# nmdp-bioinformatics/py-graph-imputation

Measured on AMD Instinct MI355X. Metric: imputed subjects/sec (whole node), 5-locus CAU graph, higher is better.
Workload: dtype f64; 1 GPU; BASELINE configs[1]: CAU 5-locus graph, 10k synthetic fully-typed subjects; 10000 subjects per step and GPU, seed=rank; graph_nodes=35411, populations=1

## Files before the change

py-graph-imputation_amd/csrc/grim_engine.hip:

```cpp
#include <hip/hip_runtime.h>
#include <hip/hip_ext.h>
#include <stdio.h>
#include <stdlib.h>
#include <string.h>
#include <algorithm>
#include <atomic>
#include <mutex>
#include <string>
#include <vector>

#include "grim_plan_a.h"
#include "grim_plan_b.h"
#include "grim_small.h"
#include "grim_medium.h"
#include "grim_mid.h"
#include "grim_tables.h"
#include "grim_tokdev.h"
#include "grim_em.h"
#include "grim_refresh.h"
#include "grim_marginal.h"
#include "grim_match.h"
#include "grim_search.h"
#include "grim_engine_internal.h"
#include "grim_host_internal.h"
// ... 492 lines not shown
  g->rf_short.clear();
  g->rf_long.clear();
  uint32_t pos = 0;
  for (uint32_t v = 0; v < V; ++v) {
    const uint32_t m = d->node_mask[v];
    if (m == d->full_mask) continue;
    const std::string node = "partial node " + std::to_string(v);
    if (m >= (1u << GRIM_MAXL)) return no(node + ": label mask beyond GRIM_MAXL");
    const uint32_t lo = d->a_start[v], hi = v + 1 < V ? d->a_start[v + 1] : n_a;
    if (lo != pos) return no(node + ": its top-link row does not begin where the row before it ends");
    if (hi <= lo) return no(node + ": empty top-link row");
    if (hi > n_a) return no(node + ": its top-link row ends beyond the links");
    for (uint32_t e = lo; e < hi; ++e) {
      const uint32_t r = d->a_nbr[e];
      if (r >= V || d->node_mask[r] != d->full_mask) return no(node + ": a top link that does not end at a full node");
      if ((d->node_key[r] & slots[m]) != d->node_key[v]) return no(node + ": a top link to a full haplotype that does not project onto it");
    }
    (hi - lo <= RF_SHORT_MAX ? g->rf_short : g->rf_long).push_back(v);
    pos = hi;
  }
  if (pos != n_a) return no("top links beyond the rows of the partial nodes");
  g->refreshable = true;
  g->refresh_why.clear();
  g->n_a_nbr = n_a;
  g->full_first = f_lo;
  g->n_full = f_hi - f_lo;
}

extern "C" grim_graph *grim_graph_upload(grim_ctx *c, const grim_graph_desc *d) {
  if (!c || !d) return nullptr;
  hipSetDevice(c->device);
  if (d->n_pops == 0 || d->n_pops > GRIM_MAXPOP) { set_err(c, "grim_graph_upload: population count out of range"); return nullptr; }
  if (d->n_loci == 0 || d->n_loci > GRIM_MAXL) { set_err(c, "grim_graph_upload: locus count out of range"); return nullptr; }
  if (d->n_nodes >= (1u << 23)) { set_err(c, "grim_graph_upload: more than 2^23 nodes"); return nullptr; }
  grim_graph *g = new grim_graph();
  g->ctx = c;
  g->bytes = 0;
  uint32_t cap = 64;
  static const int ht_factor = getenv("GRIM_HT_FACTOR") ? atoi(getenv("GRIM_HT_FACTOR")) : 0;
  while (cap < (uint64_t)(ht_factor > 1 ? ht_factor : (d->n_nodes > (1u << 18) ? 4 : 2)) * (uint64_t)d->n_nodes) cap <<= 1;
  std::vector<uint64_t> hk(cap, 0);
  std::vector<uint32_t> hv(cap, 0);
  bool unique_names = true;
  for (uint32_t i = 0; i < d->n_nodes; ++i) {
    uint64_t k = d->node_key[i];
    if (k == 0) { set_err(c, "grim_graph_upload: node with empty key"); delete g; return nullptr; }
    uint32_t h = (uint32_t)host_mix64(k) & (cap - 1);
    while (hk[h] != 0 && hk[h] != k) h = (h + 1) & (cap - 1);
    if (hk[h] == k) unique_names = false;
    hk[h] = k;
    hv[h] = i;
  }
  uint32_t max_deg = 0;
  for (uint32_t i = 0; i < d->n_nodes; ++i)
    if (d->a_start[i + 1] > d->a_start[i]) max_deg = std::max(max_deg, d->a_start[i + 1] - d->a_start[i]);
  uint32_t maxlab = 0;
  for (uint32_t m = 0; m < (1u << GRIM_MAXL); ++m) {
    uint32_t n = d->lab_start[m + 1] - d->lab_start[m];
    if (n > maxlab) maxlab = n;
  }
  g->max_label = maxlab;
  DevGraph &D = g->d;
  D.n_nodes = d->n_nodes;
  D.P = d->n_pops;
  D.n_loci = d->n_loci;
  D.full_mask = d->full_mask;
  D.ht_mask = cap - 1;
  D.n_conn = d->n_conn;
  D.node_key = upload(c, g->bufs, d->node_key, d->n_nodes, &g->bytes);
  D.node_mask = upload(c, g->bufs, d->node_mask, d->n_nodes, &g->bytes);
  D.freq = upload(c, g->bufs, d->freq, (size_t)d->n_nodes * d->n_pops, &g->bytes);
  D.a_start = upload(c, g->bufs, d->a_start, (size_t)d->n_nodes + 1, &g->bytes);
  D.a_nbr = upload(c, g->bufs, d->a_nbr, d->n_a_nbr, &g->bytes);
  D.b_conn = upload(c, g->bufs, d->b_conn, (size_t)d->n_nodes * GRIM_MAXL, &g->bytes);
  D.b_start = upload(c, g->bufs, d->b_start, (size_t)d->n_conn + 1, &g->bytes);
  D.b_nbr = upload(c, g->bufs, d->b_nbr, d->n_b_nbr, &g->bytes);
  D.lab_start = upload(c, g->bufs, d->lab_start, (1u << GRIM_MAXL) + 1, &g->bytes);
  D.lab_nodes = upload(c, g->bufs, d->lab_nodes, d->n_nodes, &g->bytes);
  {
    std::vector<uint64_t> lk(d->n_nodes);
    for (uint32_t i = 0; i < d->n_nodes; ++i) lk[i] = d->node_key[d->lab_nodes[i]];
    D.lab_key = upload(c, g->bufs, lk.data(), d->n_nodes, &g->bytes);
  }
  D.scan_ok = (unique_names && max_deg < (1u << 22) && d->n_pops <= 64) ? 1u : 0u;
  D.order_bad = d->label_order_bad;
  {
    std::vector<HtEnt> ht(cap);
    for (uint32_t i = 0; i < cap; ++i) {
      ht[i].key = hk[i];
      ht[i].val = hv[i];
      ht[i].pad = 0;
    }
    D.ht = upload(c, g->bufs, ht.data(), cap, &g->bytes);
  }
  {
    uint32_t nfull = d->lab_start[d->full_mask + 1] - d->lab_start[d->full_mask];
    uint32_t fcap = 64;
    static const int fht_factor = getenv("GRIM_FHT_FACTOR") ? atoi(getenv("GRIM_FHT_FACTOR")) : 8;
    while (fcap < (uint64_t)(fht_factor > 1 ? fht_factor : 2) * (uint64_t)nfull) fcap <<= 1;
    std::vector<FullEnt> ft(fcap);
    memset(ft.data(), 0, sizeof(FullEnt) * fcap);
    for (uint32_t i = 0; i < d->n_nodes; ++i) {
      if (d->node_mask[i] != d->full_mask) continue;
      uint64_t k = d->node_key[i];
      uint32_t h = fht_hash(k) & (fcap - 1);
      while (ft[h].key != 0 && ft[h].key != k) h = (h + 1) & (fcap - 1);
      ft[h].key = k;
      ft[h].f0 = d->freq[(size_t)i * d->n_pops];
    }
    D.fht = upload(c, g->bufs, ft.data(), fcap, &g->bytes);
    D.fht_mask = fcap - 1;
  }
  if (!D.fht || !D.node_key || !D.node_mask || !D.freq || !D.a_start || !D.a_nbr || !D.b_conn || !D.b_start || !D.b_nbr ||
      !D.lab_start || !D.lab_nodes || !D.lab_key || !D.ht) {
    set_err(c, "grim_graph_upload: device allocation or copy failed");
    for (void *p : g->bufs) hipFree(p);
    delete g;
    return nullptr;
  }
  refresh_check_rows(g, d);
  return g;
}

static void refresh_state_free(RefreshState *rf);

extern "C" void grim_graph_free(grim_graph *g) {
  if (!g) return;
  hipSetDevice(g->ctx->device);
  refresh_state_free(g->rf);
  for (void *p : g->bufs) hipFree(p);
  delete g;
}

extern "C" uint64_t grim_graph_device_bytes(const grim_graph *g) { return g ? g->bytes : 0; }


static uint64_t align256(uint64_t x) { return (x + 255) & ~255ull; }

static thread_local int tl_device = -1;
static inline void use_device(int dev) {
  if (tl_device != dev) {
    hipSetDevice(dev);
    tl_device = dev;
  }
}

static int env_int(const char *name, int dflt) {
  const char *v = getenv(name);
  return v ? atoi(v) : dflt;
}

uint32_t engine_small_stride(const grim_params *p) { return GRIM_SMALL_ROWS_FIXED + (p->n_results < 16 ? p->n_results : 16); }

uint64_t engine_rows_per_subject(const grim_params *p, uint32_t P) {
  return 2ull * p->n_results + 2ull * (p->n_pop_results < (uint64_t)P * P ? p->n_pop_results : (uint64_t)P * P);
}

static bool dev_realloc(uint8_t *&ptr, uint64_t bytes) {
  if (ptr) hipFree(ptr);
  ptr = nullptr;
  return hipMalloc((void **)&ptr, bytes ? bytes : 256) == hipSuccess;
}
static bool pin_realloc(uint8_t *&ptr, uint64_t bytes) {
  if (ptr) hipHostFree(ptr);
  ptr = nullptr;
  return hipHostMalloc((void **)&ptr, bytes ? bytes : 256, hipHostMallocDefault) == hipSuccess;
}

static std::atomic<uint64_t> g_moved[2];

static bool batch_plan(grim_batch *b, const EnginePlan &pl) {
  const uint64_t n = pl.n_subj ? pl.n_subj : 1;
  uint64_t o = 0;
  auto take = [&](uint64_t bytes) { uint64_t r = o; o = align256(o + bytes); return r; };
  const uint64_t o_state = take(8ull * (GRIM_NCTR + GRIM_NQ / 2));
  const bool devtok = pl.text_cap != 0;
  const uint64_t o_lines = take(devtok ? sizeof(LineRec) * n : 0), o_text = take(devtok ? pl.text_cap + 64 : 0);
  const uint64_t o_subj = take(sizeof(grim_subject) * n);
  const uint64_t o_small = take(sizeof(SmallRec) * n);
  const uint64_t o_os = take(4 * n), o_om = take(4 * n), o_og = take(4 * n);
  const uint64_t o_tok = take(2 * ((pl.tok_cap ? pl.tok_cap : 1) + (devtok ? (uint64_t)TOK_LANES * n : 0)));
  const uint64_t in_bytes = o;
  o = 0;
  const uint64_t small_waves = ((n + GRIM_WG / 32 - 1) / (GRIM_WG / 32)) * (GRIM_WG / 64);
  const uint64_t w_bail = take(4 * n), w_next = take(4 * n), w_ctr = take(4 * (4 * small_waves + 4));
  const uint64_t w_mid = take(4 * n);
  const uint64_t w_dsmall = take(devtok ? sizeof(SmallRec) * n : 0);
  const uint64_t w_t1 = take(sizeof(TabWork) * 2 * n), w_t2 = take(sizeof(TabWork) * 2 * n);
  const uint64_t work_bytes = o;
  o = 0;
  const uint64_t o_res = take(sizeof(grim_subject_result) * n);
  const uint64_t o_rows = take(sizeof(grim_row) * b->row_limit);
  const uint64_t out_bytes = o;
  bool ok = true;
  if (in_bytes > b->in_cap || !b->d_in) {
    const uint64_t want = in_bytes > b->in_cap ? in_bytes : b->in_cap;
    ok = ok && dev_realloc(b->d_in, want) && pin_realloc(b->h_in, want);
    b->in_cap = ok ? want : 0;
  }
  if (work_bytes > b->work_cap || !b->d_work) {
    const uint64_t want = work_bytes > b->work_cap ? work_bytes : b->work_cap;
    ok = ok && dev_realloc(b->d_work, want);
    b->work_cap = ok ? want : 0;
  }
  if (out_bytes > b->out_cap || !b->d_out) {
    const uint64_t want = out_bytes > b->out_cap ? out_bytes : b->out_cap;
    ok = ok && dev_realloc(b->d_out, want);
    b->out_cap = ok ? want : 0;
  }
  if (!ok) return false;
  b->plan = pl;
  b->off_tok = o_tok;
  b->off_rows = o_rows;
  DevArgs &A = b->a;
  A.counters = (unsigned long long *)(b->d_in + o_state);
  A.queue = (uint32_t *)(A.counters + GRIM_NCTR);
  A.row_head = A.queue + 1;
  A.next_count = A.queue + 2;
  A.subj = (const grim_subject *)(b->d_in + o_subj);
  b->d_small = (SmallRec *)(b->d_in + o_small);
  b->d_lines = devtok ? (LineRec *)(b->d_in + o_lines) : nullptr;
  b->d_text = devtok ? b->d_in + o_text : nullptr;
  b->d_dsmall = devtok ? (SmallRec *)(b->d_work + w_dsmall) : nullptr;
  b->off_subj = o_subj;
  b->h.lines = devtok ? (LineRec *)(b->h_in + o_lines) : nullptr;
  b->h.text = devtok ? b->h_in + o_text : nullptr;
  b->d_os = (uint32_t *)(b->d_in + o_os);
  b->d_om = (uint32_t *)(b->d_in + o_om);
  A.order = (const uint32_t *)(b->d_in + o_og);
  A.tok = (const uint16_t *)(b->d_in + o_tok);
  A.bail_list = (uint32_t *)(b->d_work + w_bail);
  A.next_list = (uint32_t *)(b->d_work + w_next);
  {
    static const int no_mid = env_int("GRIM_NO_MID", 0);
    A.mid_list = no_mid ? nullptr : (uint32_t *)(b->d_work + w_mid);
  }
  A.small_ctr = (uint32_t *)(b->d_work + w_ctr);
  A.t1_list = (TabWork *)(b->d_work + w_t1);
  A.t2_list = (TabWork *)(b->d_work + w_t2);
  A.res = (grim_subject_result *)(b->d_out + o_res);
  A.rows = (grim_row *)(b->d_out + o_rows);
  A.row_cap = (uint32_t)b->row_limit;
  A.priors = b->d_priors;
  A.next_cap = (uint32_t)n;
  b->h.subj = (grim_subject *)(b->h_in + o_subj);
  b->h.small = (SmallRec *)(b->h_in + o_small);
  b->h.order_s = (uint32_t *)(b->h_in + o_os);
  b->h.order_m = (uint32_t *)(b->h_in + o_om);
  b->h.order_g = (uint32_t *)(b->h_in + o_og);
  b->h.tok = (uint16_t *)(b->h_in + o_tok);
  b->h.res = (grim_subject_result *)b->h_out;
  b->h.rows = (grim_row *)(b->h_out ? b->h_out + o_rows : nullptr);
  return true;
}

static void batch_init_params(grim_batch *b, const grim_graph *g, const grim_params *p) {
  b->g = g;
  DevArgs &A = b->a;
  A.g = g->d;
  A.prm = *p;
  const uint32_t P = g->d.P;
  b->small_stride = engine_small_stride(p);
  A.pair_cap = GRIM_MAXPH * p->top_n * p->top_n;
  uint32_t tab = 64;
  while (tab < 2 * A.pair_cap) tab <<= 1;
  A.tab_cap = tab;
  A.bset_cap = g->max_label;
  SlotLayout &L = A.lay;
  uint64_t o = 0;
  auto take = [&](uint64_t n) { uint64_t r = o; o = align256(o + n); return r; };
  L.Tp = take(8ull * GRIM_SIDES * GRIM_TOPCAP);
  L.Tm = take(8ull * GRIM_SIDES * GRIM_TOPCAP);
  L.Te = take(4ull * GRIM_SIDES * GRIM_TOPCAP);
  L.k0 = take(8ull * tab);
  L.k1 = take(8ull * tab);
  L.tmin = take(4ull * tab);
  L.tgid = take(4ull * tab);
  L.Useq = take(4ull * A.pair_cap);
  L.Uprob = take(8ull * A.pair_cap);
  L.Uslot = take(4ull * A.pair_cap);
  L.ska = take(8ull * A.pair_cap);
  L.skb = take(8ull * A.pair_cap);
  L.sva = take(4ull * A.pair_cap);
  L.svb = take(4ull * A.pair_cap);
  L.gsum = take(8ull * A.pair_cap);
  L.ghead = take(4ull * A.pair_cap);
  L.gstart = take(4ull * (A.pair_cap + 1));
  L.gcnt = take(4ull * (A.pair_cap > P * P ? A.pair_cap : P * P));
  L.qsum = take(8ull * P * P);
  L.qfirst = take(4ull * P * P);
  L.bset = take(4ull * GRIM_NWAVE * GRIM_MAXL * (uint64_t)A.bset_cap);
  L.comp = take(8ull * GRIM_COMP_CAP);
  {
    uint32_t pc = 64;
    while (pc < 2 * A.bset_cap) pc <<= 1;
    A.proj_cap = pc;
  }
  L.proj_k = take(8ull * GRIM_NWAVE * A.proj_cap);
  L.proj_p = take(4ull * GRIM_NWAVE * A.proj_cap);
  L.rtok = take(2ull * GRIM_RTOK_CAP);
  L.save = take(p->save_mode ? 8ull * GRIM_NWAVE * 2 * GRIM_SAVE_CAP * (P + 1) : 0);
  L.stride = align256(o);
  b->timing = env_int("GRIM_TIMING", 0) != 0;
  A.flags = (env_int("GRIM_TABLES_HBM", 0) ? GRIM_F_TABLES_HBM : 0u) | (env_int("GRIM_NO_NODUP", 0) ? GRIM_F_NO_NODUP : 0u) |
            (env_int("GRIM_NO_SIDEMASK", 0) ? GRIM_F_NO_SIDEMASK : 0u);
  memset(b->acc_ms, 0, sizeof(b->acc_ms));
  b->n_timed = 0;
  b->n_subj = b->n_small = b->n_medium = b->n_general = 0;
  b->rows_used = 0;
}

grim_batch *engine_batch_create(grim_ctx *c, const grim_graph *g, const grim_params *p, uint64_t row_limit, const EnginePlan *plan) {
  if (!c || !g || !p || !plan) return nullptr;
  use_device(c->device);
  if (p->top_n == 0 || p->top_n > GRIM_TOPCAP) { set_err(c, "grim_batch_upload: max_haplotypes_number_in_phase must be 1..128"); return nullptr; }
  if (p->n_ladder < 0 || p->n_ladder > GRIM_MAXLADDER) { set_err(c, "grim_batch_upload: epsilon ladder too long"); return nullptr; }
  if (row_limit > 0x7FFFFFF0ull) row_limit = 0x7FFFFFF0ull;
  if (row_limit < 64) row_limit = 64;
  grim_batch *b = nullptr;
  if (!c->spare.empty()) {
    b = c->spare.back();
    c->spare.pop_back();
    if (b->d_priors) hipFree(b->d_priors);
    if (b->h_priors) hipHostFree(b->h_priors);
    b->d_priors = b->h_priors = nullptr;
    b->priors_cap = b->priors_up = 0;
  } else {
    b = new grim_batch();
    memset((void *)b, 0, sizeof(*b));
    b->ctx = c;
    bool ok = true;
    if (hipHostMalloc((void **)&b->hstate, 8 * (GRIM_NCTR + GRIM_NQ / 2)) != hipSuccess) {
      b->hstate = nullptr;
      ok = false;
    }
    for (auto &pair : b->ev)
      for (hipEvent_t &e : pair) ok = ok && hipEventCreate(&e) == hipSuccess;
    ok = ok && hipEventCreateWithFlags(&b->ev_done, hipEventDisableTiming | hipEventReleaseToSystem) == hipSuccess;
// ... 62 lines not shown
  use_device(c->device);
  grim_devdict *dd = new grim_devdict();
  dd->ctx = c;
  memset(&dd->d, 0, sizeof(dd->d));
  dd->d.n_loci = snap->n_loci;
  for (uint32_t s = 0; s < GRIM_MAXL; ++s) dd->d.locus_len[s] = 0xFFFFFFFFu;
  for (const DictSnap::Locus &L : snap->loci) {
    if (L.slot >= GRIM_MAXL || L.name.empty() || L.name.size() > 8) continue;
    uint64_t v = 0;
    for (size_t k = 0; k < L.name.size(); ++k) v |= (uint64_t)(uint8_t)L.name[k] << (56 - 8 * k);
    dd->d.locus[L.slot] = v;
    dd->d.locus_len[L.slot] = (uint32_t)L.name.size();
  }
  bool ok = true;
  for (uint32_t s = 0; s < snap->n_loci && s < GRIM_MAXL && ok; ++s) {
    const uint32_t cnt = snap->base[s];
    uint32_t cap = 16;
    while (cap < 4ull * cnt) cap <<= 1;
    std::vector<DictEnt> tab(cap);
    memset(tab.data(), 0, sizeof(DictEnt) * cap);
    for (uint32_t id = 0; id < cnt; ++id) {
      const sv nm = snap->name(s, id);
      if (nm.empty() || nm.size() > GRIM_TOKNAME) continue;
      DictEnt e;
      pack_name(nm.data(), nm.size(), e.w);
      e.hash = tokname_hash(e.w, (uint32_t)nm.size());
      e.meta = 0x80000000u | ((uint32_t)nm.size() << 16) | (id & 0xFFFFu);
      uint32_t k = e.hash & (cap - 1);
      while (tab[k].meta >> 31) k = (k + 1) & (cap - 1);
      tab[k] = e;
    }
    DictEnt *dt = upload(c, dd->bufs, tab.data(), cap, nullptr);
    ok = dt != nullptr;
    dd->d.tab[s] = dt;
    dd->d.mask[s] = cap - 1;
  }
  if (!ok) {
    set_err(c, "engine_devdict_create: device allocation or copy failed");
    engine_devdict_free(dd);
    return nullptr;
  }
  return dd;
}

void engine_devdict_free(grim_devdict *d) {
  if (!d) return;
  use_device(d->ctx->device);
  for (void *p : d->bufs) hipFree(p);
  delete d;
}

void engine_batch_set_dict(grim_batch *b, const grim_devdict *d) {
  if (b) b->dict = d;
}

uint32_t engine_batch_irregular(const grim_batch *b) { return b ? b->n_irregular : 0; }
uint32_t engine_graph_order_bad(const grim_graph *g) { return g ? g->d.order_bad : 0; }

int engine_batch_grow_pool(grim_batch *b, uint64_t max_records) {
  if (!b || b->pool_asked <= b->a.ppool_cap) return 0;
  uint64_t want = b->pool_asked + b->pool_asked / 8 + 4096;
  if (want > max_records || want > 0x7FFFFFF0ull) return 0;
  if (want <= b->pool_want) return 0;
  b->pool_want = want;
  return 1;
}

static int batch_set_rows(grim_batch *b, uint64_t rows) {
  const uint64_t old = b->row_limit;
  b->row_limit = rows;
  const EnginePlan pl = b->plan;
  if (!batch_plan(b, pl)) {
    (void)hipGetLastError();
    b->row_limit = old;
    if (!batch_plan(b, pl)) set_err(b->ctx, "grim_batch: device allocation failed while growing the row pool");
    return 0;
  }
  return 1;
}
int engine_batch_grow_rows(grim_batch *b, uint64_t max_rows) {
  if (!b || b->rows_used < b->a.row_cap || b->row_limit >= max_rows) return 0;
  use_device(b->ctx->device);
  uint64_t want = b->row_limit * 2;
  if (want > max_rows) want = max_rows;
  if (want > 0x7FFFFFF0ull) want = 0x7FFFFFF0ull;
  if (want <= b->row_limit) return 0;
  return batch_set_rows(b, want);
}
uint64_t engine_batch_row_limit(const grim_batch *b) { return b ? b->row_limit : 0; }
void engine_batch_hint_rows(grim_batch *b, uint64_t rows) {
  if (!b || rows <= b->row_limit) return;
  use_device(b->ctx->device);
  (void)batch_set_rows(b, rows);
}

uint64_t engine_batch_pool_want(const grim_batch *b) { return b ? b->pool_want : 0; }
void engine_batch_hint_pool(grim_batch *b, uint64_t records) {
  if (b && records > b->pool_want) b->pool_want = records;
}

int engine_batch_load(grim_batch *b, const EngineLoad *ld) {
  if (!b || !ld) return -1;
  grim_ctx *c = b->ctx;
  use_device(c->device);
  DevArgs &A = b->a;
  b->ran_ok = false;
  if (ld->n_subj > b->plan.n_subj || ld->tok_used > b->plan.tok_cap) {
    set_err(c, "engine_batch_load: beyond what the batch was planned for");
    return -1;
  }
  hipStream_t st = c->stream;
  const uint32_t P = b->g->d.P;
  const uint64_t PP = (uint64_t)P * P;
  if (ld->priors && (ld->n_priors != b->priors_up || !b->d_priors)) {
    if (ld->n_priors + 1 > b->priors_cap || !b->d_priors) {
      const uint32_t want = ld->n_priors + 1 > 2 * b->priors_cap ? ld->n_priors + 1 : 2 * b->priors_cap;
      if (b->d_priors) hipFree(b->d_priors);
      if (b->h_priors) hipHostFree(b->h_priors);
      b->d_priors = b->h_priors = nullptr;
      if (hipMalloc((void **)&b->d_priors, 8 * (uint64_t)want * PP) != hipSuccess ||
          hipHostMalloc((void **)&b->h_priors, 8 * (uint64_t)want * PP, hipHostMallocDefault) != hipSuccess) {
        set_err(c, "engine_batch_load: allocation of the prior matrices failed");
        return -1;
      }
      b->priors_cap = want;
    }
    if (ld->n_priors) memcpy(b->h_priors, ld->priors, 8 * (uint64_t)ld->n_priors * PP);
    for (uint64_t k = 0; k < PP; ++k) b->h_priors[(uint64_t)ld->n_priors * PP + k] = 1.0;
    HIPCHK(hipMemcpyAsync(b->d_priors, b->h_priors, 8 * ((uint64_t)ld->n_priors + 1) * PP, hipMemcpyHostToDevice, st), c, -1);
    g_moved[0] += 8 * ((uint64_t)ld->n_priors + 1) * PP;
    b->priors_up = ld->n_priors;
  }
  A.priors = b->d_priors;
  A.ones_prior = b->priors_up;
  if (ld->dev_hi > ld->dev_lo && (!b->dict || !b->d_lines || ld->text_bytes > b->plan.text_cap || ld->dev_hi > ld->n_subj)) {
    set_err(c, "engine_batch_load: the batch was not planned for the device tokenizer");
    return -1;
  }
  b->dev_lo = ld->dev_lo;
  b->dev_hi = ld->dev_hi;
  b->n_dev_lines = ld->dev_hi > ld->dev_lo ? ld->dev_hi - ld->dev_lo : 0;
  b->n_irregular = 0;
  b->n_subj = ld->n_subj;
  b->n_small = ld->n_small;
  b->n_medium = ld->n_medium;
  b->n_general = ld->n_general;
  b->last_load = *ld;
  b->last_load.priors = nullptr;
  A.n_medium = ld->n_medium;
  A.n_work = ld->n_general;
  unsigned long long *hs = (unsigned long long *)b->h_in;
  memset(hs, 0, 8 * (GRIM_NCTR + GRIM_NQ / 2));
  {
    const uint64_t staged = ((uint64_t)b->n_small + b->n_dev_lines) * b->small_stride;
    A.row_cap = (uint32_t)(b->row_limit - (staged <= b->row_limit ? staged : 0));
  }
  const bool host_subjects = ld->n_small + ld->n_medium + ld->n_general > 0;
  const uint64_t bytes = (!host_subjects && b->n_dev_lines) ? b->off_subj : b->off_tok + 2 * ld->tok_used;
  HIPCHK(hipMemcpyAsync(b->d_in, b->h_in, bytes, hipMemcpyHostToDevice, c->up_stream), c, -1);
  HIPCHK(hipEventRecord(b->ev_up, c->up_stream), c, -1);
  b->up_pending = true;
  g_moved[0] += bytes;
  {
    uint64_t R = (1ull << 20) + 512ull * ((uint64_t)ld->n_medium + ld->n_general) + 16ull * ld->n_small;
    R += (uint64_t)(ld->n_general < 256u ? ld->n_general : 256u) * (A.pair_cap / 2);
    const char *env_pool = getenv("GRIM_PAIR_POOL");
    if (env_pool && atol(env_pool) > 0) R = (uint64_t)atol(env_pool);
    if (b->pool_want > R) R = b->pool_want;
    if (R > 0x7FFFFFF0ull) R = 0x7FFFFFF0ull;
    const uint64_t items = 2ull * ld->n_subj < R / 256 + 1 ? 2ull * ld->n_subj : R / 256 + 1;
    uint64_t cap_b = R / 4 + (items + 1) * ((uint64_t)P * P + 4), cap_u = R / 4 + items * 64 + 1024;
    if (cap_b > R + 4096) cap_b = R + 4096;
    uint64_t o = 0;
    auto take = [&](uint64_t bytes) { uint64_t r = o; o = align256(o + bytes); return r; };
    const uint64_t o_pool = take(sizeof(PairRec) * R), o_aux = take(sizeof(TabAux) * 2 * (uint64_t)(ld->n_subj ? ld->n_subj : 1)),
                   o_boff = take(4 * cap_b), o_cell = take(sizeof(CellRec) * cap_b), o_units = take(sizeof(TabUnit) * cap_u),
                   o_sort = take(4 * 3 * R), o_grp = take(sizeof(GrpRec) * 2 * R), o_prob = take(8 * R);
    if (o > b->pool_bytes || !b->d_pool) {
      HIPCHK(hipStreamSynchronize(st), c, -1);
      if (b->d_pool) hipFree(b->d_pool);
      b->d_pool = nullptr;
      b->pool_bytes = 0;
      if (hipMalloc((void **)&b->d_pool, o) != hipSuccess) {
        (void)hipGetLastError();
        set_err(c, "engine_batch_load: cannot allocate " + std::to_string((unsigned long long)(o >> 20)) + " MiB for the table kernels");
        return -1;
      }
      b->pool_bytes = o;
    }
    b->pool_cap = R;
    A.ppool = (PairRec *)(b->d_pool + o_pool);
    A.ppool_cap = (uint32_t)R;
    A.taux = (TabAux *)(b->d_pool + o_aux);
    A.tboff = (uint32_t *)(b->d_pool + o_boff);
    A.tcell = (CellRec *)(b->d_pool + o_cell);
    A.tboff_cap = (uint32_t)cap_b;
    A.tunits = (TabUnit *)(b->d_pool + o_units);
    A.tunits_cap = (uint32_t)cap_u;
    A.tstride = (uint32_t)R;
    A.psort = (uint32_t *)(b->d_pool + o_sort);
    A.pgrp = (GrpRec *)(b->d_pool + o_grp);
    A.pprob = (double *)(b->d_pool + o_prob);
  }
  const uint32_t per_block = GRIM_WG / 32;
  b->n_host_small_waves = ((b->n_small + per_block - 1) / per_block) * (GRIM_WG / 64);
  b->n_small_waves = b->n_host_small_waves + ((b->n_dev_lines + per_block - 1) / per_block) * (GRIM_WG / 64);
  uint32_t slots = (uint32_t)c->n_cu * GRIM_WG_PER_CU;
  static const int env_slots = env_int("GRIM_SLOTS", 0);
  if (env_slots > 0) slots = (uint32_t)env_slots;
  if (slots > ld->n_subj) slots = ld->n_subj;
  if (slots == 0) slots = 1;
  b->n_slots = slots;
  b->scratch_need = (uint64_t)A.lay.stride * slots;
  if (b->gexec) {
    hipGraphExecDestroy(b->gexec);
    b->gexec = nullptr;
  }
  b->graph_state = 0;
  b->rows_used = 0;
  b->small_ctr_pending = false;
  return 0;
}

extern "C" grim_batch *grim_batch_upload(grim_ctx *c, const grim_graph *g, const grim_params *p, const grim_batch_desc *d) {
  if (!c || !g || !p || !d) return nullptr;
  use_device(c->device);
  const uint32_t P = g->d.P;
  ClassRule rule;
  rule.small_ok = (P == 1) && p->opt_threshold > 1 && !getenv("GRIM_NO_SMALL") && g->d.order_bad == 0;
  rule.medium_ok = !getenv("GRIM_NO_MEDIUM") && g->d.order_bad == 0;
  rule.medium_max_cost = getenv("GRIM_MEDIUM_MAXCOST") ? atof(getenv("GRIM_MEDIUM_MAXCOST")) : 0.0;
  rule.graph_loci = g->d.n_loci;
  rule.opt_threshold = p->opt_threshold;
  std::vector<uint32_t> os, om, og;
  for (uint32_t i = 0; i < d->n_subjects; ++i) {
    const int cls = grim_classify(rule, d->subjects[i]);
    (cls == GRIM_CLS_SMALL ? os : cls == GRIM_CLS_MEDIUM ? om : og).push_back(i);
  }
  {
    std::vector<double> cs(d->n_subjects);
    for (uint32_t i : og) cs[i] = grim_cost(d->subjects[i]);
    std::stable_sort(og.begin(), og.end(), [&](uint32_t a, uint32_t b2) { return cs[a] > cs[b2]; });
  }
  const uint64_t per = engine_rows_per_subject(p, P);
  uint64_t want = per * d->n_subjects + per * om.size() + 2ull * engine_small_stride(p) * os.size() + 1024 +
                  (uint64_t)GRIM_ROW_GRAB * c->n_cu * 32;
  const char *env_rows = getenv("GRIM_ROW_CAP");
  if (env_rows) want = strtoull(env_rows, nullptr, 10);
  if (want > 0x7FFFFFF0ull) want = 0x7FFFFFF0ull;
  EnginePlan plan{d->n_subjects ? d->n_subjects : 1u, d->n_tokens ? d->n_tokens : 1ull};
  grim_batch *b = engine_batch_create(c, g, p, want, &plan);
  if (!b) return nullptr;
  if (d->n_subjects) memcpy(b->h.subj, d->subjects, sizeof(grim_subject) * (size_t)d->n_subjects);
  if (d->n_tokens) memcpy(b->h.tok, d->tokens, 2 * (size_t)d->n_tokens);
  for (size_t k = 0; k < os.size(); ++k) {
    const grim_subject &sj = d->subjects[os[k]];
    grim_small_rec(sj, d->tokens + sj.tok_off, os[k], b->h.small[k]);
    b->h.order_s[k] = os[k];
  }
  if (!om.empty()) memcpy(b->h.order_m, om.data(), 4 * om.size());
  if (!og.empty()) memcpy(b->h.order_g, og.data(), 4 * og.size());
  std::vector<double> one_prior;
  const double *pri = d->priors;
  if (!d->n_priors) {
    one_prior.assign((size_t)P * P, 1.0);
    pri = one_prior.data();
  }
  EngineLoad ld{d->n_subjects, (uint32_t)os.size(), (uint32_t)om.size(), (uint32_t)og.size(), d->n_tokens,
                d->n_priors ? d->n_priors : 1u, pri};
  const int lrc = engine_batch_load(b, &ld);
  if (lrc != 0 || hipStreamSynchronize(c->stream) != hipSuccess) {
    if (lrc == 0) set_err(c, "grim_batch_upload: copy failed");
    grim_batch_free(b);
    return nullptr;
  }
  return b;
}

static int bind_scratch(grim_batch *b) {
  grim_ctx *c = b->ctx;
  if (b->scratch_need > c->scratch_bytes) {
    if (c->scratch) {
      hipStreamSynchronize(c->stream);
      hipFree(c->scratch);
    }
    c->scratch = nullptr;
    c->scratch_bytes = 0;
    if (hipMalloc(&c->scratch, b->scratch_need) != hipSuccess) {
      (void)hipGetLastError();
      set_err(c, "grim_batch_run: cannot allocate " + std::to_string((unsigned long long)(b->scratch_need >> 20)) + " MiB of scratch");
      return -1;
    }
    c->scratch_bytes = b->scratch_need;
  }
  b->a.scratch = (uint8_t *)c->scratch;
  b->a.wctr = c->wctr;
  return 0;
}

template <typename... P, typename... Q>
static void launch_span(grim_batch *b, Phase ph, bool start, bool stop, void (*kernel)(P...), dim3 grid, dim3 block, Q &&...args) {
  if (b->timing && ph != PH_NONE) {
    b->launched |= 1u << ph;
    hipExtLaunchKernelGGL(kernel, grid, block, 0, b->ctx->stream, start ? b->ev[ph][0] : nullptr, stop ? b->ev[ph][1] : nullptr, 0,
                          static_cast<P>(args)...);
  } else {
    hipLaunchKernelGGL(kernel, grid, block, 0, b->ctx->stream, static_cast<P>(args)...);
  }
}
template <typename... P, typename... Q>
static void launch(grim_batch *b, Phase ph, void (*kernel)(P...), dim3 grid, dim3 block, Q &&...args) {
  launch_span(b, ph, true, true, kernel, grid, block, args...);
}

static void enqueue_tables(grim_batch *b) {
  grim_ctx *c = b->ctx;
  DevArgs &A = b->a;
  const uint32_t cand = b->n_subj;
  uint32_t g1 = (uint32_t)c->n_cu * 14u, g2 = (uint32_t)c->n_cu * GRIM_TAB_WG_PER_CU;
  if (g1 > cand) g1 = cand;
  if (g2 > b->n_slots) g2 = b->n_slots;
  if (g1 == 0) g1 = 1;
  if (g2 == 0) g2 = 1;
  static int bucket_per_cu = 0;
  if (bucket_per_cu == 0) {
    int nb = 0;
    if (hipOccupancyMaxActiveBlocksPerMultiprocessor(&nb, grim_tables_bucket_kernel, 64, 0) != hipSuccess || nb <= 0) {
      (void)hipGetLastError();
      nb = 8;
    }
    bucket_per_cu = nb > 32 ? 32 : nb;
  }
  const uint32_t g3 = (uint32_t)c->n_cu * (uint32_t)bucket_per_cu;
  uint32_t g4 = (uint32_t)c->n_cu * (160u * 1024u / (uint32_t)sizeof(SplitWave)), g5 = (uint32_t)c->n_cu * 16u;
  if (g4 > cand) g4 = cand;
  if (g5 > cand) g5 = cand;
  if (g4 == 0) g4 = 1;
  if (g5 == 0) g5 = 1;
  (void)hipMemsetAsync(c->wctr, 0, 4 * GRIM_WCTR_WORDS, c->stream);
  launch_span(b, PH_TABLES, true, false, grim_tables_wave_kernel, dim3(g1), dim3(64), A);
  launch(b, PH_NONE, grim_tables_split_wave_kernel, dim3(g4), dim3(64), A);
  launch(b, PH_NONE, grim_tables_split_kernel, dim3(g2), dim3(GRIM_WG), A);
  launch(b, PH_NONE, grim_tables_bucket_kernel, dim3(g3), dim3(64), A);
  launch(b, PH_NONE, grim_tables_merge_wave_kernel, dim3(g5), dim3(64), A);
  launch_span(b, PH_TABLES, false, true, grim_tables_merge_kernel, dim3(g2), dim3(GRIM_WG), A);
}

static void enqueue_half_wave(grim_batch *b, bool timed, const DevArgs &Ak, const SmallRec *recs, const uint32_t *order, uint32_t n, uint32_t stage) {
  const uint32_t per_block = GRIM_WG / 32;
  launch(b, timed ? PH_HALF_WAVE : PH_NONE, grim_plan_a_small_kernel, dim3((n + per_block - 1) / per_block), dim3(GRIM_WG), Ak, recs, n, stage,
         b->small_stride);
  launch(b, timed ? PH_COMPACT : PH_NONE, grim_small_compact_kernel, dim3((n + 63) / 64), dim3(64), b->a, order, order ? nullptr : recs, n, stage,
         b->small_stride);
}

static int enqueue_stage1(grim_batch *b) {
  grim_ctx *c = b->ctx;
  DevArgs &A = b->a;
  const uint32_t stage0 = (uint32_t)b->row_limit - (b->n_small + b->n_dev_lines) * b->small_stride;
  if (b->n_small) enqueue_half_wave(b, b->n_dev_lines == 0, A, b->d_small, b->d_os, b->n_small, stage0);
  if (b->n_dev_lines) {
    DevTok T;
    T.text = b->d_text;
    T.lines = b->d_lines;
    T.lo = b->dev_lo;
    T.hi = b->dev_hi;
    T.dict = b->dict->d;
    T.dsmall = b->d_dsmall;
    T.subj = const_cast<grim_subject *>(A.subj);
    T.tok = const_cast<uint16_t *>(A.tok);
    T.tok_base = (uint32_t)(b->plan.tok_cap ? b->plan.tok_cap : 1);
    T.graph_loci = A.g.n_loci;
    const dim3 tgrid((b->n_dev_lines + (GRIM_WG / 64) * TOK_LINES_PER_WAVE - 1) / ((GRIM_WG / 64) * TOK_LINES_PER_WAVE));
    launch(b, PH_TOKENIZER, grim_tokenize_kernel, tgrid, dim3(GRIM_WG), A, T);
    DevArgs A2 = A;
    A2.small_ctr = A.small_ctr + 2 * b->n_host_small_waves;
    enqueue_half_wave(b, true, A2, b->d_dsmall, nullptr, b->n_dev_lines, stage0 + b->n_small * b->small_stride);
  }
  if (b->n_medium) {
    static const int waves_per_cu = env_int("GRIM_MEDIUM_WAVES", GRIM_MEDIUM_WAVES_PER_CU);
    uint32_t grid = (uint32_t)c->n_cu * (uint32_t)(waves_per_cu > 0 ? waves_per_cu : GRIM_MEDIUM_WAVES_PER_CU);
    if (grid > b->n_medium) grid = b->n_medium;
    launch(b, PH_ONE_WAVE, grim_plan_a_medium_kernel, dim3(grid), dim3(64), A, b->d_om, b->n_medium, A.bail_list);
  }
  if (A.mid_list && b->n_general + b->n_medium) {
    const uint32_t want = b->n_general + b->n_medium;
    uint32_t grid = (uint32_t)c->n_cu * GRIM_MID_WG_PER_CU;
    if (grid > want) grid = want;
    launch(b, PH_MID, grim_plan_a_mid_kernel, dim3(grid), dim3(GRIM_WG), A);
  }
  if (b->n_general + b->n_medium) {
    uint32_t want = b->n_general + b->n_medium;
    launch(b, PH_GENERAL, grim_plan_a_kernel, dim3(b->n_slots < want ? b->n_slots : want), dim3(GRIM_WG), A);
  }
  launch(b, PH_NONE, grim_finish_kernel, dim3(1), dim3(GRIM_WG), A.counters, b->hstate, 0u, 0);
  return hipGetLastError() == hipSuccess ? 0 : -1;
}

extern "C" int grim_batch_set_timing(grim_batch *b, int on) {
  if (!b) return -1;
  b->timing = on != 0;
  memset(b->acc_ms, 0, sizeof(b->acc_ms));
  b->n_timed = 0;
  return 0;
}

int engine_batch_upload_done(grim_batch *b) {
  if (!b || !b->up_pending) return 1;
  use_device(b->ctx->device);
  if (hipEventQuery(b->ev_up) == hipSuccess) return 1;
  (void)hipGetLastError();
  return 0;
}

int engine_batch_enqueue(grim_batch *b) {
  if (!b) return -1;
  grim_ctx *c = b->ctx;
  use_device(c->device);
  if (((uint64_t)b->n_small + b->n_dev_lines) * b->small_stride > b->row_limit) {
    b->rows_used = 0;
    set_err(c, "grim_batch_run: output row pool smaller than the half-wave kernel's fixed region");
    return -2;
  }
  memset(b->ms, 0, sizeof(b->ms));
  b->launched = 0;
  std::lock_guard<std::mutex> lk(c->run_mu);
  if (bind_scratch(b) != 0) return -1;
  if (b->up_pending) {
    b->up_pending = false;
    if (hipEventQuery(b->ev_up) != hipSuccess) {
      (void)hipGetLastError();
      HIPCHK(hipStreamWaitEvent(c->stream, b->ev_up, 0), c, -1);
    }
  }
  if (b->timing) {
    if (enqueue_stage1(b) != 0) {
      set_err(c, "grim_batch_run: kernel launch failed");
      return -1;
    }
  } else {
    if (b->graph_state == 0) {
      b->graph_state = -1;
      static const int use_graph = env_int("GRIM_GRAPH", 0);
      if (use_graph && hipStreamBeginCapture(c->stream, hipStreamCaptureModeThreadLocal) == hipSuccess) {
        int rc = enqueue_stage1(b);
        hipGraph_t gr = nullptr;
        hipError_t e = hipStreamEndCapture(c->stream, &gr);
        if (rc == 0 && e == hipSuccess && gr && hipGraphInstantiate(&b->gexec, gr, nullptr, nullptr, 0) == hipSuccess)
          b->graph_state = 1;
        if (gr) hipGraphDestroy(gr);
        (void)hipGetLastError();
      }
    }
    if (b->graph_state == 1) {
      HIPCHK(hipGraphLaunch(b->gexec, c->stream), c, -1);
    } else if (enqueue_stage1(b) != 0) {
      set_err(c, "grim_batch_run: kernel launch failed");
      return -1;
    }
  }
  HIPCHK(hipEventRecord(b->ev_done, c->stream), c, -1);
  b->enqueued = true;
  return 0;
}

static int read_phase_times(grim_batch *b) {
  for (int p = 0; p < PH_COUNT; ++p)
    if (b->launched >> p & 1) HIPCHK(hipEventElapsedTime(&b->ms[p], b->ev[p][0], b->ev[p][1]), b->ctx, -1);
  b->launched = 0;
  return 0;
}

int engine_batch_wait(grim_batch *b) {
  if (!b) return -1;
  grim_ctx *c = b->ctx;
  use_device(c->device);
  DevArgs &A = b->a;
  if (!b->enqueued) {
    set_err(c, "engine_batch_wait: nothing in flight");
    return -1;
  }
  b->enqueued = false;
  b->ran_ok = false;
  HIPCHK(hipEventSynchronize(b->ev_done), c, -1);
  if (read_phase_times(b) != 0) return -1;
  uint32_t head[GRIM_NQ];
  memcpy(head, b->hstate + GRIM_NCTR, 4 * GRIM_NQ);
  const bool run_b = A.prm.planb && head[2] + head[6] > 0;
  if (run_b || head[2] + head[6] + head[9] + head[10] > 0) {
    {
      std::lock_guard<std::mutex> lk(c->run_mu);
      if (bind_scratch(b) != 0) return -1;
      if (run_b) {
        uint32_t grid = b->n_slots < head[2] + head[6] ? b->n_slots : head[2] + head[6];
        launch(b, PH_PLAN_B, grim_plan_b_kernel, dim3(grid), dim3(GRIM_WG), A);
        if (hipGetLastError() != hipSuccess) {
          set_err(c, "grim_batch_run: plan-B launch failed");
          return -1;
        }
      }
      enqueue_tables(b);
      launch(b, PH_NONE, grim_finish_kernel, dim3(1), dim3(GRIM_WG), A.counters, b->hstate, 0u, 1);
      HIPCHK(hipGetLastError(), c, -1);
      HIPCHK(hipEventRecord(b->ev_done, c->stream), c, -1);
    }
    HIPCHK(hipEventSynchronize(b->ev_done), c, -1);
    if (read_phase_times(b) != 0) return -1;
    memcpy(head, b->hstate + GRIM_NCTR, 4 * GRIM_NQ);
  }
  if (b->timing) {
    for (int p = 0; p < PH_COUNT; ++p) b->acc_ms[p] += b->ms[p];
    b->n_timed++;
  }
  static const int dbg_classes = env_int("GRIM_DEBUG_CLASSES", 0);
  if (dbg_classes)
    fprintf(stderr, "grim classes: mid-size kernel took %u, handed %u to the general kernel\n", head[16], head[17]);
  if (dbg_classes)
    fprintf(stderr, "grim classes: small %u medium %u general %u | medium->general %u (+%u heavier), to plan B %u (+%u heavy) | table items %u one-wave, %u bigger (%u work units), %u pair records; workgroup merge: %u items (%u with an overflowed bucket), up to %u pairs; workgroup split: %u items | stage 1 %s\n",
            b->n_small, b->n_medium, b->n_general, head[5], head[7], head[2], head[6], head[9], head[10], head[14], head[8], head[21], head[22], head[23], head[12],
            b->graph_state == 1 ? "replayed as a hipGraph" : "launched directly");
  memcpy(b->counters, b->hstate, 64);
  b->small_ctr_pending = b->n_small + b->n_dev_lines > 0;
  for (int sh = 0; sh < 64; ++sh)
    for (int k = 0; k < 3; ++k) b->counters[k] += b->hstate[8 + 4 * sh + k];
  b->rows_used = head[1];
  b->pool_asked = head[8];
  b->n_irregular = head[GRIM_Q_IRREGULAR];
#ifdef GRIM_STAMPS
  fprintf(stderr, "grim stamps (us):");
  for (int k = 0; k < 16; ++k) fprintf(stderr, " [%d]%.0f", k, b->hstate[GRIM_STAMP_BASE + k] / 100.0);
  fprintf(stderr, "\n");
  fprintf(stderr, "grim mid-size kernel stage us (setup, probes, rows, entries, lists, ladder, first pass, final pass, emit):");
  for (int k = 0; k < 9; ++k) fprintf(stderr, " %.0f", b->hstate[GRIM_MID_BASE + k] / 100.0);
  fprintf(stderr, "\ngrim mid-size kernel hand-overs (branch/candidates, hits, rows, entries, lists, pairs, dedup):");
  for (int k = 0; k < 7; ++k) fprintf(stderr, " %llu", b->hstate[GRIM_MID_BASE + 16 + k]);
  fprintf(stderr, "\n");
  static const char *hname[8] = {"0", "1", "2", "3 workgroup-merge items by pairs", "4 workgroup-split items by pairs",
                                 "5 workgroup-split us by pairs", "6 workgroup-merge items by genotype groups",
                                 "7 workgroup-merge us by pairs"};
  for (int h = 0; h < 8; ++h) {
    fprintf(stderr, "grim hist %s:", hname[h]);
    for (int k = 0; k < 24; ++k) fprintf(stderr, " %llu", b->hstate[GRIM_HIST_BASE + 24 * h + k]);
    fprintf(stderr, "\n");
  }
#endif
  if (b->counters[4] != 0 || head[1] > A.row_cap) {
    if (b->rows_used > A.row_cap) b->rows_used = A.row_cap;
    set_err(c, "grim_batch_run: output row pool exhausted (raise GRIM_ROW_CAP or lower the batch size)");
    return -2;
  }
  b->ran_ok = true;
  return 0;
}

extern "C" int grim_batch_run(grim_batch *b) {
  if (!b) return -1;
  int rc = engine_batch_enqueue(b);
  if (rc == 0) rc = engine_batch_wait(b);
  if (rc == -2 && !b->in_retry && engine_batch_grow_pool(b, 256ull << 20)) {
    b->in_retry = true;
    EngineLoad ld = b->last_load;
    rc = engine_batch_load(b, &ld);
    if (rc == 0) rc = grim_batch_run(b);
    b->in_retry = false;
  }
  return rc;
}

extern "C" int grim_batch_run_repeat(grim_batch *b, uint32_t n) {
  for (uint32_t i = 0; i < n; ++i) {
    const int rc = grim_batch_run(b);
    if (rc != 0) return rc;
// ... 1342 lines not shown
```

py-graph-imputation_amd/csrc/grim_small.h:

```cpp
#pragma once
#include "grim_pair.h"


__device__ __forceinline__ double half_shfl_d(double v, int src_in_half) {
  return __shfl(v, (threadIdx.x & 32) | src_in_half);
}
__device__ __forceinline__ uint32_t half_shfl_u(uint32_t v, int src_in_half) {
  return __shfl(v, (threadIdx.x & 32) | src_in_half);
}

template <int CTRL>
__device__ __forceinline__ double dpp_d(double v) {
  const long long b = __double_as_longlong(v);
  const int lo = __builtin_amdgcn_update_dpp(0, (int)(uint32_t)b, CTRL, 0xF, 0xF, false);
  const int hi = __builtin_amdgcn_update_dpp(0, (int)(uint32_t)((unsigned long long)b >> 32), CTRL, 0xF, 0xF, false);
  return __longlong_as_double((long long)(((unsigned long long)(uint32_t)hi << 32) | (uint32_t)lo));
}
__device__ __forceinline__ double row16_max(double v) {
  double o;
  o = dpp_d<0x121>(v); v = o > v ? o : v;
  o = dpp_d<0x122>(v); v = o > v ? o : v;
  o = dpp_d<0x124>(v); v = o > v ? o : v;
  o = dpp_d<0x128>(v); v = o > v ? o : v;
  return v;
}

__global__ __launch_bounds__(GRIM_WG) void grim_plan_a_small_kernel(DevArgs A, const SmallRec *recs, uint32_t n,
                                                                   uint32_t row_base, uint32_t row_stride) {
  const DevGraph &g = A.g;
  const int hl = threadIdx.x & 31;
  const uint32_t w = blockIdx.x * (GRIM_WG / 32) + (threadIdx.x >> 5);
  bool live = w < n;
  const int n_ladder = A.prm.n_ladder;
  double lad[8];
#pragma unroll
  for (int i = 0; i < 8; ++i) lad[i] = A.prm.ladder[i];
  bool hit = false;
  uint64_t mykey = 0;
  double f = 0.0;
  uint32_t same = 0, si = 0;
  double w_prior = 0.0;
  if (live) {
    const uint4 *rp = (const uint4 *)(recs + w);
    const uint4 r0 = rp[0], r1 = rp[1];
    const uint32_t words[8] = {r0.x, r0.y, r0.z, r0.w, r1.x, r1.y, r1.z, r1.w};
    same = (words[6] >> 8) & 0xFFu;
    si = words[7];
    live = si != GRIM_NONE;
    w_prior = live ? A.priors[(uint64_t)(words[6] >> 16)] : 0.0;
#pragma unroll
    for (int l = 0; l < GRIM_MAXL; ++l) {
      const uint32_t tw = words[l];
      const uint32_t t = ((hl >> l) & 1) ? (tw >> 16) : (tw & 0xFFFFu);
      const uint32_t slot = (l < 4 ? (words[5] >> (8 * l)) : words[6]) & 0xFFu;
      mykey |= (uint64_t)(t + 1u) << (GRIM_ABITS * slot);
    }
    uint32_t h = fht_hash(mykey) & g.fht_mask;
    for (; live;) {
      const FullEnt e = g.fht[h];
      if (e.key == mykey) { hit = true; f = e.f0; break; }
      if (e.key == 0) break;
      h = (h + 1) & g.fht_mask;
    }
  }
  const bool hit2 = half_shfl_u(hit ? 1u : 0u, hl ^ 31) != 0;
  const double f2 = half_shfl_d(f, hl ^ 31);
  const uint64_t key2 = ((uint64_t)half_shfl_u((uint32_t)(mykey >> 32), hl ^ 31) << 32) | half_shfl_u((uint32_t)mykey, hl ^ 31);
  const uint32_t het4 = 15u & ~same;
  bool kept = hl < 16 && ((uint32_t)hl & ~het4 & 15u) == 0 && (!((same >> 4) & 1u) || ((uint32_t)hl ^ het4) >= (uint32_t)hl);
  const bool pair_ok = live && kept && f > 0.0 && f2 > 0.0;
  const bool same_hap = mykey == key2;
  PairRef pr;
  pr.p1 = f; pr.p2 = f2; pr.m2 = f2;
  pr.e1 = same_hap ? 0u : 1u; pr.e2 = 0u;
  const bool hi_half = (threadIdx.x & 32) != 0;
  double eps = 0.0;
  bool found = false;
  bool acc = false;
  {
    const uint64_t okb = __ballot(pair_ok);
    bool need_lo = (okb & 0xFFFFull) != 0, need_hi = ((okb >> 32) & 0xFFFFull) != 0;
    bool got_lo = false, got_hi = false;
    double eps_lo = 0.0, eps_hi = 0.0;
    auto step = [&](double e) {
      const bool a = pair_ok && pair_accept(e, pr, w_prior);
      const uint64_t b = __ballot(a);
      const bool take_lo = need_lo && (b & 0xFFFFull), take_hi = need_hi && ((b >> 32) & 0xFFFFull);
      if (take_lo) { need_lo = false; got_lo = true; eps_lo = e; }
      if (take_hi) { need_hi = false; got_hi = true; eps_hi = e; }
      if (hi_half ? take_hi : take_lo) acc = a;
    };
#pragma unroll
    for (int idx = 0; idx < 8; ++idx)
      if (idx < n_ladder && (need_lo || need_hi)) step(lad[idx]);
    for (int idx = 8; idx < n_ladder && (need_lo || need_hi); ++idx) step(A.prm.ladder[idx]);
    eps = hi_half ? eps_hi : eps_lo;
    found = hi_half ? got_hi : got_lo;
  }
  double prob = acc ? pair_prob(pr, w_prior) : 0.0;
  double mx = row16_max(prob);
  if (found && eps > 0.0) {
    eps = mx / 100000.0;
    acc = pair_ok && pair_accept(eps, pr, w_prior);
    prob = acc ? pair_prob(pr, w_prior) : 0.0;
    mx = row16_max(prob);
  }
  const uint64_t bal = __ballot(acc);
  const uint32_t accmask = (uint32_t)(hi_half ? (bal >> 32) : bal) & 0xFFFFu;
  const uint32_t nU = __popc(accmask);
  double total = 0.0;
  bool first = true;
  uint32_t rank = 0;
  for (uint32_t um = ((uint32_t)bal | (uint32_t)(bal >> 32)) & 0xFFFFu; um; um &= um - 1) {
    const int i = __builtin_ctz(um);
    const double p_lo = lane_get(prob, i), p_hi = lane_get(prob, 32 + i);
    const double pi = hi_half ? p_hi : p_lo;
    if ((accmask >> i) & 1u) {
      total = first ? pi : total + pi;
      first = false;
      if (pi > prob || (pi == prob && i < hl)) ++rank;
    }
  }
  {
    const uint64_t need = __ballot(live && kept), needp = __ballot(live && kept && hit),
                   needq = __ballot(live && kept && hit2);
    if ((threadIdx.x & 63) == 0) {
      const uint32_t gw = blockIdx.x * (GRIM_WG / 64) + (threadIdx.x >> 6);
      *(uint2 *)(A.small_ctr + 2 * gw) = make_uint2(2u * (uint32_t)__popcll(need), (uint32_t)(__popcll(needp) + __popcll(needq)));
    }
  }
  if (!live) return;
  const uint32_t off = row_base + w * row_stride;
  const bool ok = nU > 0;
  const int first_lane = ok ? (__ffs(accmask) - 1) : 0;
  const uint32_t n_pm = (ok && A.prm.out_haps) ? (nU < A.prm.n_results ? nU : A.prm.n_results) : 0;
  const uint64_t ka = ((uint64_t)half_shfl_u((uint32_t)(mykey >> 32), first_lane) << 32) | half_shfl_u((uint32_t)mykey, first_lane);
  const uint64_t kb = ((uint64_t)half_shfl_u((uint32_t)(key2 >> 32), first_lane) << 32) | half_shfl_u((uint32_t)key2, first_lane);
  {
    const int f = hl - 16;
    const bool phase = hl < 16;
    const bool wr = ok && (phase ? (acc && rank < n_pm) : f == 0);
    if (wr) {
      grim_row r;
      r.a = phase ? mykey : ka;
      r.b = phase ? key2 : kb;
      r.prob = phase ? prob : total;
      r.popa = 0;
      r.popb = 0;
      A.rows[off + (phase ? GRIM_SMALL_ROWS_FIXED + rank : (uint32_t)f)] = r;
    }
  }
  if (hl >= 19 && hl < 26) {
    const int j = hl - 19;
    const uint8_t status = ok ? GRIM_ST_OK : (A.prm.planb ? GRIM_ST_UNSUPPORTED : GRIM_ST_MISS);
    const uint32_t head = (uint32_t)status | ((uint32_t)'a' << 8) | ((!ok && A.prm.planb) ? (2u << 16) : 0u);
    const uint32_t n_um = (ok && A.prm.out_muug && A.prm.n_results) ? 1u : 0u;
    const uint32_t n_up = (ok && A.prm.out_muug && A.prm.n_pop_results) ? 1u : 0u;
    const uint32_t n_pp = (ok && A.prm.out_haps && A.prm.n_pop_results) ? 1u : 0u;
    const uint64_t mxb = ok ? (uint64_t)__double_as_longlong(mx) : 0ull;
    uint32_t lo, hi;
    switch (j) {
      case 0: lo = head; hi = ok ? nU : 0u; break;
      case 1: lo = ok ? 1u : 0u; hi = ok ? off + 0 : 0u; break;
      case 2: lo = ok ? off + 0 : 0u; hi = ok ? off + GRIM_SMALL_ROWS_FIXED : 0u; break;
      case 3: lo = ok ? off + 0 : 0u; hi = n_um; break;
      case 4: lo = n_up; hi = n_pm; break;
      case 5: lo = n_pp; hi = 0u; break;
      default: lo = (uint32_t)mxb; hi = (uint32_t)(mxb >> 32); break;
    }
    ((uint2 *)(A.res + si))[j] = make_uint2(lo, hi);
  }
  if (!ok && hl == 0 && A.prm.planb) push_next(A, si, false);
}
```

Measured before the change: 145.2 million subjects/s.

## Compact device-tokenized small-subject rows via workgroup atomic placement

Device-tokenized small subjects now go through a new place kernel. It computes each subject's actual row count, does a workgroup prefix sum in shared memory and takes a single atomicAdd on the shared row head, instead of writing into a fixed per-subject strided region reserved at the end of the row pool. This shrinks the staged fixed region, so the row pool is not padded per device line, and it packs output rows densely to cut memory footprint and downstream copy volume. In exchange it adds __syncthreads and a global atomic per 1024-thread workgroup, and the row order is no longer deterministic.

New measurement: 140.7 million subjects/s. -3.1%, worse.

```diff
diff --git a/py-graph-imputation_amd/csrc/grim_engine.hip b/py-graph-imputation_amd/csrc/grim_engine.hip
--- a/py-graph-imputation_amd/csrc/grim_engine.hip
+++ b/py-graph-imputation_amd/csrc/grim_engine.hip
@@ -668,6 +668,11 @@
 
 uint32_t engine_small_stride(const grim_params *p) { return GRIM_SMALL_ROWS_FIXED + (p->n_results < 16 ? p->n_results : 16); }
 
+static uint32_t place_waves(uint32_t n) {
+  const uint32_t per_block = GRIM_SMALL_PLACE_WG / 32;
+  return ((n + per_block - 1) / per_block) * (GRIM_SMALL_PLACE_WG / 64);
+}
+
 uint64_t engine_rows_per_subject(const grim_params *p, uint32_t P) {
   return 2ull * p->n_results + 2ull * (p->n_pop_results < (uint64_t)P * P ? p->n_pop_results : (uint64_t)P * P);
 }
@@ -699,7 +704,7 @@
   const uint64_t in_bytes = o;
   o = 0;
   const uint64_t small_waves = ((n + GRIM_WG / 32 - 1) / (GRIM_WG / 32)) * (GRIM_WG / 64);
-  const uint64_t w_bail = take(4 * n), w_next = take(4 * n), w_ctr = take(4 * (4 * small_waves + 4));
+  const uint64_t w_bail = take(4 * n), w_next = take(4 * n), w_ctr = take(4 * (4 * small_waves + 4 + 2 * (GRIM_SMALL_PLACE_WG / 64)));
   const uint64_t w_mid = take(4 * n);
   const uint64_t w_dsmall = take(devtok ? sizeof(SmallRec) * n : 0);
   const uint64_t w_t1 = take(sizeof(TabWork) * 2 * n), w_t2 = take(sizeof(TabWork) * 2 * n);
@@ -1068,7 +1073,7 @@
   unsigned long long *hs = (unsigned long long *)b->h_in;
   memset(hs, 0, 8 * (GRIM_NCTR + GRIM_NQ / 2));
   {
-    const uint64_t staged = ((uint64_t)b->n_small + b->n_dev_lines) * b->small_stride;
+    const uint64_t staged = (uint64_t)b->n_small * b->small_stride;
     A.row_cap = (uint32_t)(b->row_limit - (staged <= b->row_limit ? staged : 0));
   }
   const bool host_subjects = ld->n_small + ld->n_medium + ld->n_general > 0;
@@ -1120,7 +1125,7 @@
   }
   const uint32_t per_block = GRIM_WG / 32;
   b->n_host_small_waves = ((b->n_small + per_block - 1) / per_block) * (GRIM_WG / 64);
-  b->n_small_waves = b->n_host_small_waves + ((b->n_dev_lines + per_block - 1) / per_block) * (GRIM_WG / 64);
+  b->n_small_waves = b->n_host_small_waves + place_waves(b->n_dev_lines);
   uint32_t slots = (uint32_t)c->n_cu * GRIM_WG_PER_CU;
   static const int env_slots = env_int("GRIM_SLOTS", 0);
   if (env_slots > 0) slots = (uint32_t)env_slots;
@@ -1273,7 +1278,7 @@
 static int enqueue_stage1(grim_batch *b) {
   grim_ctx *c = b->ctx;
   DevArgs &A = b->a;
-  const uint32_t stage0 = (uint32_t)b->row_limit - (b->n_small + b->n_dev_lines) * b->small_stride;
+  const uint32_t stage0 = (uint32_t)b->row_limit - b->n_small * b->small_stride;
   if (b->n_small) enqueue_half_wave(b, b->n_dev_lines == 0, A, b->d_small, b->d_os, b->n_small, stage0);
   if (b->n_dev_lines) {
     DevTok T;
@@ -1291,7 +1296,9 @@
     launch(b, PH_TOKENIZER, grim_tokenize_kernel, tgrid, dim3(GRIM_WG), A, T);
     DevArgs A2 = A;
     A2.small_ctr = A.small_ctr + 2 * b->n_host_small_waves;
-    enqueue_half_wave(b, true, A2, b->d_dsmall, nullptr, b->n_dev_lines, stage0 + b->n_small * b->small_stride);
+    const uint32_t per_block = GRIM_SMALL_PLACE_WG / 32;
+    launch(b, PH_HALF_WAVE, grim_plan_a_small_place_kernel, dim3((b->n_dev_lines + per_block - 1) / per_block), dim3(GRIM_SMALL_PLACE_WG), A2,
+           b->d_dsmall, b->n_dev_lines);
   }
   if (b->n_medium) {
     static const int waves_per_cu = env_int("GRIM_MEDIUM_WAVES", GRIM_MEDIUM_WAVES_PER_CU);
@@ -1333,7 +1340,7 @@
   if (!b) return -1;
   grim_ctx *c = b->ctx;
   use_device(c->device);
-  if (((uint64_t)b->n_small + b->n_dev_lines) * b->small_stride > b->row_limit) {
+  if ((uint64_t)b->n_small * b->small_stride > b->row_limit) {
     b->rows_used = 0;
     set_err(c, "grim_batch_run: output row pool smaller than the half-wave kernel's fixed region");
     return -2;
diff --git a/py-graph-imputation_amd/csrc/grim_small.h b/py-graph-imputation_amd/csrc/grim_small.h
--- a/py-graph-imputation_amd/csrc/grim_small.h
+++ b/py-graph-imputation_amd/csrc/grim_small.h
@@ -1,5 +1,7 @@
 #pragma once
 #include "grim_pair.h"
+
+#define GRIM_SMALL_PLACE_WG 1024
 
 
 __device__ __forceinline__ double half_shfl_d(double v, int src_in_half) {
@@ -25,11 +27,12 @@
   return v;
 }
 
-__global__ __launch_bounds__(GRIM_WG) void grim_plan_a_small_kernel(DevArgs A, const SmallRec *recs, uint32_t n,
-                                                                   uint32_t row_base, uint32_t row_stride) {
+template <bool PLACE, int WG>
+__device__ __forceinline__ void plan_a_small_body(const DevArgs &A, const SmallRec *recs, uint32_t n, uint32_t row_base,
+                                                  uint32_t row_stride) {
   const DevGraph &g = A.g;
   const int hl = threadIdx.x & 31;
-  const uint32_t w = blockIdx.x * (GRIM_WG / 32) + (threadIdx.x >> 5);
+  const uint32_t w = blockIdx.x * (WG / 32) + (threadIdx.x >> 5);
   bool live = w < n;
   const int n_ladder = A.prm.n_ladder;
   double lad[8];
@@ -125,21 +128,58 @@
     const uint64_t need = __ballot(live && kept), needp = __ballot(live && kept && hit),
                    needq = __ballot(live && kept && hit2);
     if ((threadIdx.x & 63) == 0) {
-      const uint32_t gw = blockIdx.x * (GRIM_WG / 64) + (threadIdx.x >> 6);
+      const uint32_t gw = blockIdx.x * (WG / 64) + (threadIdx.x >> 6);
       *(uint2 *)(A.small_ctr + 2 * gw) = make_uint2(2u * (uint32_t)__popcll(need), (uint32_t)(__popcll(needp) + __popcll(needq)));
     }
   }
+  const bool ok = nU > 0;
+  const uint32_t n_pm = (ok && A.prm.out_haps) ? (nU < A.prm.n_results ? nU : A.prm.n_results) : 0;
+  const uint32_t n_um = (ok && A.prm.out_muug && A.prm.n_results) ? 1u : 0u;
+  const uint32_t n_up = (ok && A.prm.out_muug && A.prm.n_pop_results) ? 1u : 0u;
+  const uint32_t n_pp = (ok && A.prm.out_haps && A.prm.n_pop_results) ? 1u : 0u;
+  uint32_t off;
+  bool rows_ok = true;
+  if (PLACE) {
+    const uint32_t cnt = (n_um | n_up | n_pm | n_pp) ? GRIM_SMALL_ROWS_FIXED + n_pm : 0u;
+    __shared__ uint32_t wave_cnt[WG / 64];
+    __shared__ uint32_t run_base;
+    const uint32_t c_lo = __shfl(cnt, 0), c_hi = __shfl(cnt, 32);
+    const uint32_t wv = threadIdx.x >> 6;
+    if ((threadIdx.x & 63) == 0) wave_cnt[wv] = c_lo + c_hi;
+    __syncthreads();
+    uint32_t before = 0, wg_rows = 0;
+#pragma unroll
+    for (uint32_t k = 0; k < WG / 64; ++k) {
+      const uint32_t c = wave_cnt[k];
+      before += k < wv ? c : 0u;
+      wg_rows += c;
+    }
+    if (threadIdx.x == 0) {
+      uint32_t base = 0;
+      if (wg_rows) {
+        base = atomicAdd(A.row_head, wg_rows);
+        if (base + wg_rows > A.row_cap) {
+          atomicExch(&A.counters[4], 1ull);
+          base = GRIM_NONE;
+        }
+      }
+      run_base = base;
+    }
+    __syncthreads();
+    const uint32_t base = run_base;
+    rows_ok = base != GRIM_NONE && cnt != 0;
+    off = base + before + (hi_half ? c_lo : 0u);
+  } else {
+    off = row_base + w * row_stride;
+  }
   if (!live) return;
-  const uint32_t off = row_base + w * row_stride;
-  const bool ok = nU > 0;
   const int first_lane = ok ? (__ffs(accmask) - 1) : 0;
-  const uint32_t n_pm = (ok && A.prm.out_haps) ? (nU < A.prm.n_results ? nU : A.prm.n_results) : 0;
   const uint64_t ka = ((uint64_t)half_shfl_u((uint32_t)(mykey >> 32), first_lane) << 32) | half_shfl_u((uint32_t)mykey, first_lane);
   const uint64_t kb = ((uint64_t)half_shfl_u((uint32_t)(key2 >> 32), first_lane) << 32) | half_shfl_u((uint32_t)key2, first_lane);
   {
     const int f = hl - 16;
     const bool phase = hl < 16;
-    const bool wr = ok && (phase ? (acc && rank < n_pm) : f == 0);
+    const bool wr = ok && rows_ok && (phase ? (acc && rank < n_pm) : f == 0);
     if (wr) {
       grim_row r;
       r.a = phase ? mykey : ka;
@@ -154,9 +194,6 @@
     const int j = hl - 19;
     const uint8_t status = ok ? GRIM_ST_OK : (A.prm.planb ? GRIM_ST_UNSUPPORTED : GRIM_ST_MISS);
     const uint32_t head = (uint32_t)status | ((uint32_t)'a' << 8) | ((!ok && A.prm.planb) ? (2u << 16) : 0u);
-    const uint32_t n_um = (ok && A.prm.out_muug && A.prm.n_results) ? 1u : 0u;
-    const uint32_t n_up = (ok && A.prm.out_muug && A.prm.n_pop_results) ? 1u : 0u;
-    const uint32_t n_pp = (ok && A.prm.out_haps && A.prm.n_pop_results) ? 1u : 0u;
     const uint64_t mxb = ok ? (uint64_t)__double_as_longlong(mx) : 0ull;
     uint32_t lo, hi;
     switch (j) {
@@ -172,3 +209,12 @@
   }
   if (!ok && hl == 0 && A.prm.planb) push_next(A, si, false);
 }
+
+__global__ __launch_bounds__(GRIM_WG) void grim_plan_a_small_kernel(DevArgs A, const SmallRec *recs, uint32_t n,
+                                                                   uint32_t row_base, uint32_t row_stride) {
+  plan_a_small_body<false, GRIM_WG>(A, recs, n, row_base, row_stride);
+}
+
+__global__ __launch_bounds__(GRIM_SMALL_PLACE_WG) void grim_plan_a_small_place_kernel(DevArgs A, const SmallRec *recs, uint32_t n) {
+  plan_a_small_body<true, GRIM_SMALL_PLACE_WG>(A, recs, n, 0u, 0u);
+}
```
